# jaswon/osu-dreamer

Measured on AMD Instinct MI355X. Metric: denoiser train-steps/sec + 50-step sample latents/sec, 1/2/4/8 MI355X, higher is better.
Workload: dtype bf16

## Files before the change

### include/osu_dreamer_hip.h

```cpp
#ifndef OSU_DREAMER_HIP_H
#define OSU_DREAMER_HIP_H

#ifdef __cplusplus
extern "C" {
#endif

enum { OD_F32 = 0, OD_BF16 = 1,
       OD_F32X3 = 2,
       OD_F32X3W = 3,
       OD_F16 = 4 };
enum { OD_EPI_NONE = 0, OD_EPI_SILU = 1 };
enum { OD_ACT_NONE = 0, OD_ACT_SILU = 1 };
enum { OD_ERR_ARG = -1, OD_ERR_ALIGN = -2, OD_ERR_UNSUPPORTED = -3, OD_ERR_COMM = -4 };

int od_version(void);
const char* od_build_source_sha(void);
const char* od_error_string(int code);

int od_gemm_nt(int dtype, const void* A, int lda, const void* W, int ldw, const float* bias, void* C, int ldc,
               int M, int N, int K, int epilogue, int accumulate, void* stream);
int od_gemm_nt_qkrope(int dtype, const void* A, int lda, const void* W, int ldw, const float* bias, void* C, int ldc, int M,
                      int N, int K, const float* wq, const float* wk, const float* table, int L, int H, int hd, float eps,
                      float q_scale, void* stream);
int od_gemm_nt_qkrope_split(int dtype, const void* A, int lda, const void* W, int ldw, const float* bias, void* C, int ldc,
                            void* qk_out, int ldqk, int qk_dtype, int M, int N, int K, const float* wq, const float* wk, const float* table,
                            int L, int H, int hd, float eps, float q_scale, void* stream);
int od_gemm_tn(int dtype, const void* G, int ldg, const void* A, int lda, float* dW, int lddw, float* dbias, int M, int N,
               int K, void* stream);
int od_gemm_tn_blocks(int dtype, const void* G, int ldg, const void* A, int lda, float* dW, int lddw, float* dbias, int M, int N,
                      int K, int n_block, int n_valid, void* stream);
int od_colsum(int dtype, const void* G, int ldg, float* out, int M, int N, void* stream);
int od_pack_weight(int dtype, const float* src, int N, int K, void* dst, int Np, int Kp, int transpose,
                   const int* row_map, void* stream);

int od_linear_small(const float* x, const float* W, const float* b, float* out, float* pre, int B, int N, int K, int act,
                    void* stream);
int od_linear_small_bwd(const float* x, const float* W, const float* pre, const float* dout, float* dpre, float* dW,
                        float* db, float* dx, int accumulate_dx, int B, int N, int K, int act, void* stream);

int od_cl_to_frames(int dtype, const float* src, void* dst, int ldd, int B, int C, int L, void* stream);
int od_feed_gather(const float* store, long store_elems, const long* base, const long* cstride, const int* lens, float* out,
                   int N, int C, int Lpad, void* stream);
int od_proj_in(int dtype, const float* xt, const float* W, const float* bias, void* x, int ldx, int B, int E, int L,
               int D, void* stream);
int od_proj_in_bwd(int dtype, const float* xt, const void* dx, int ldx, float* dW, float* db, int B, int E, int L, int D,
                   void* stream);
int od_silu(int dtype, const void* x, void* y, long n, void* stream);
int od_silu_bwd(int dtype, const void* x, const void* dy, void* dx, long n, void* stream);

int od_rmsnorm_film(int dtype, const void* x, int ldx, const float* ssg, const void* cl, int ldcl, int cl_bcast,
                    void* h, int ldh, float* inv_rms, int B, int L, int C, float eps, void* stream);
int od_rmsnorm_film_bwd(int dtype, const void* x, int ldx, const float* inv_rms, const float* ssg, const void* dh,
                        int lddh, void* dres, int lddres, float* dssg, int B, int L, int C, void* stream);
int od_rmsnorm_gate_residual(int dtype, const void* x, int ldx, const void* h, int ldh, const float* ssg, void* xo,
                             int ldxo, float* inv_rms, int B, int L, int C, float eps, void* stream);
int od_rmsnorm_gate_residual_film(int dtype, const void* x, int ldx, const void* h, int ldh, const float* ssg_a, void* xo, int ldxo,
                                  float* inv_a, const float* ssg_b, const void* cl, int ldcl, int cl_bcast, void* h2, int ldh2,
                                  float* inv_b, int B, int L, int C, float eps, void* stream);
int od_rmsnorm_gate_residual_film_dwconv(int dtype, const void* x, int ldx, const void* h, int ldh, const float* ssg_a, void* xo, int ldxo,
                                         float* inv_a, const float* ssg_b, void* h2, int ldh2, float* inv_b, const float* conv_w,
                                         const float* conv_b, void* y, int ldy, int B, int L, int C, int ksize, float eps, void* stream);
int od_rmsnorm_gate_residual_bwd(int dtype, const void* h, int ldh, const float* inv_rms, const float* ssg,
                                 const void* dy, int lddy, void* dh, int lddh, float* dssg, int B, int L, int C,
                                 void* stream);

int od_rope_table(float* table, int L, int hd, void* stream);
int od_qk_norm_rope(int dtype, const void* qkv, int ldqkv, const float* wq, const float* wk, const float* table,
                    void* qk_out, int ldo, int B, int L, int H, int hd, float eps, float q_scale, void* stream);
int od_qk_norm_rope_bwd(int dtype, const void* qkv, int ldqkv, const float* wq, const float* wk, const float* table,
                        const void* dqk, int lddqk, void* dqkv, int lddqkv, float* dwq, float* dwk, int B, int L,
                        int H, int hd, float eps, float q_scale, void* stream);
int od_flash_attn_fwd(int dtype, const void* q, int ldq, const void* k, int ldk, const void* v, int ldv, void* o, int ldo,
                      float* lse, int B, int H, int L, int hd, float scale, int q_prescaled, void* stream);
int od_flash_attn_fwd_varlen(int dtype, const void* q, int ldq, const void* k, int ldk, const void* v, int ldv, void* o, int ldo,
                             float* lse, const int* lens, int B, int H, int L, int hd, float scale, int q_prescaled, void* stream);
int od_flash_attn_bwd(int dtype, const void* q, int ldq, const void* k, int ldk, const void* v, int ldv, const void* o,
                      int ldo, const void* dout, int lddo, const float* lse, float* delta, void* dq, int lddq, void* dk,
                      int lddk, void* dv, int lddv, int B, int H, int L, int hd, float scale, int q_prescaled, void* stream);
int od_attn_aux_create(void** aux_out);
int od_attn_aux_destroy(void* aux);
int od_flash_attn_bwd_aux(int dtype, const void* q, int ldq, const void* k, int ldk, const void* v, int ldv, const void* o,
                          int ldo, const void* dout, int lddo, const float* lse, float* delta, void* dq, int lddq, void* dk,
                          int lddk, void* dv, int lddv, int B, int H, int L, int hd, float scale, int q_prescaled, void* aux, void* stream);
int od_flash_attn_bwd_varlen(int dtype, const void* q, int ldq, const void* k, int ldk, const void* v, int ldv, const void* o,
                             int ldo, const void* dout, int lddo, const float* lse, float* delta, void* dq, int lddq, void* dk,
                             int lddk, void* dv, int lddv, const int* lens, int B, int H, int L, int hd, float scale, int q_prescaled,
                             void* aux, void* stream);
int od_flash_attn_bwd_fused_ws_bytes(int dtype, int B, int H, int L, long* total_out, long* zero_out);
int od_flash_attn_bwd_fused(int dtype, const void* q, int ldq, const void* k, int ldk, const void* v, int ldv, const void* o, int ldo,
                            const void* dout, int lddo, const float* lse, void* dq, int lddq, void* dk, int lddk, void* dv, int lddv,
                            int B, int H, int L, int hd, float scale, int q_prescaled, void* ws, long ws_bytes, void* stream);
int od_flash_attn_bwd_fused_status(const void* ws, int* err_out, void* stream);
int od_flash_attn_bwd_fused_err_offset(void);
int od_flash_attn_bwd_fused_passes(void);
int od_flash_attn_bwd_fused_prof(void* ws, long* out16);
int od_flash_attn_bwd_passes(void);

int od_dwconv(int dtype, const void* x, int ldx, const float* w, const float* bias, void* y, int ldy, int B, int L,
              int C, int ksize, void* stream);
int od_dwconv_varlen(int dtype, const void* x, int ldx, const float* w, const float* bias, void* y, int ldy, const int* lens,
                     int B, int L, int C, int ksize, void* stream);
int od_dwconv_bwd(int dtype, const void* x, int ldx, const float* w, const void* dy, int lddy, void* dx, int lddx,
                  float* dw, float* db, int B, int L, int C, int ksize, void* stream);
int od_dwconv_bwd_varlen(int dtype, const void* x, int ldx, const float* w, const void* dy, int lddy, void* dx, int lddx,
                         float* dw, float* db, const int* lens, int B, int L, int C, int ksize, void* stream);
int od_scale_channels(int dtype, void* x, int ldx, const float* scale, int B, int L, int C, void* stream);
int od_swiglu_rmsnorm(int dtype, const void* vg, int ldvg, void* hh, int ldhh, float* inv_rms, int M, int Hf, int Hp,
                      float eps, void* stream);
int od_swiglu_rmsnorm_bwd(int dtype, const void* vg, int ldvg, const float* inv_rms, const void* dhh, int lddhh,
                          void* dvg, int lddvg, int M, int Hf, int Hp, void* stream);

int od_final_norm_proj_out(int dtype, const void* x, int ldx, const float* W, const float* bias, float* v,
                           float* inv_rms, int B, int L, int C, int E, float eps, void* stream);
int od_final_norm_proj_out_bwd(int dtype, const void* x, int ldx, const float* inv_rms, const float* W, const float* dv,
                               void* dx, int lddx, float* dW, float* db, int B, int L, int C, int E, void* stream);
int od_uhead_fwd(const float* xt, const float* w0, const float* b0, const float* w1, const float* b1, const float* w3,
                 const float* b3, const float* w4, const float* b4, float* fsum, int B, int E, int L, int U,
// ... 157 lines not shown
```

### osu_dreamer_amd/csrc/rowops.hip

```cpp
#include "od_common.h"
#include "od_api_internal.h"

namespace {

#ifndef OD_QK_BPW
#define OD_QK_BPW 8
#endif
constexpr int ROWS_PER_WAVE_BWD = 16;

template <class T, int NCH>
__device__ __forceinline__ void load_row(const T* row, int C, int lane, float (&v)[NCH][8]) {
#pragma unroll
    for (int i = 0; i < NCH; i++) {
        const int c = (lane + 64 * i) * 8;
        if (c < C) od_ld8(row + c, v[i]);
        else {
#pragma unroll
            for (int e = 0; e < 8; e++) v[i][e] = 0.f;
        }
    }
}
template <int NCH>
__device__ __forceinline__ float row_sumsq(const float (&v)[NCH][8]) {
    float s = 0.f;
// ... 282 lines not shown
    const int b = blockIdx.y;
    const int l0 = (blockIdx.x * 4 + wave) * ROWS_PER_WAVE_BWD;
    float dg[NCH][8], gate[NCH][8];
#pragma unroll
    for (int i = 0; i < NCH; i++) {
        const int c = (lane + 64 * i) * 8;
#pragma unroll
        for (int e = 0; e < 8; e++) { dg[i][e] = 0.f; gate[i][e] = 0.f; }
        if (c < C) od_ld8(ssg + (size_t)b * 3 * C + 2 * C + c, gate[i]);
    }
    for (int r = 0; r < ROWS_PER_WAVE_BWD; r++) {
        const int l = l0 + r;
        if (l >= L) break;
        const long m = (long)b * L + l;
        float hv[NCH][8], gv[NCH][8];
        load_row<T, NCH>(h + m * ldh, C, lane, hv);
        load_row<T, NCH>(dy + m * lddy, C, lane, gv);
        const float inv = inv_rms[m];
        float dot = 0.f;
#pragma unroll
        for (int i = 0; i < NCH; i++)
#pragma unroll
            for (int e = 0; e < 8; e++) {
                const float hh = hv[i][e] * inv;
                dg[i][e] += gv[i][e] * hh;
                gv[i][e] *= gate[i][e];
                dot += gv[i][e] * hh;
                hv[i][e] = hh;
            }
        dot = od_wave_sum(dot) / (float)C;
#pragma unroll
        for (int i = 0; i < NCH; i++) {
            const int c = (lane + 64 * i) * 8;
            if (c >= C) continue;
            float o[8];
#pragma unroll
            for (int e = 0; e < 8; e++) o[e] = inv * (gv[i][e] - hv[i][e] * dot);
            od_st8(dh + m * lddh + c, o);
        }
    }
    for (int w = 0; w < 4; w++) {
        if (wave == w) {
#pragma unroll
            for (int i = 0; i < NCH; i++)
#pragma unroll
                for (int e = 0; e < 8; e++) {
                    const int idx = (lane + 64 * i) * 8 + e;
                    if (w == 0) red[idx] = dg[i][e]; else red[idx] += dg[i][e];
                }
        }
        __syncthreads();
    }
    for (int c = threadIdx.x; c < C; c += 256) od_red_add(det, dssg + (size_t)b * 3 * C + 2 * C + c, red[c]);
}

template <class T, int NCH>
__global__ __launch_bounds__(256) void swiglu_rmsnorm_kernel(const T* __restrict__ vg, int ldvg, T* __restrict__ hh, int ldhh,
                                                             float* __restrict__ inv_rms, long M, int Hf, int Hp, float eps) {
    const int lane = threadIdx.x & 63;
    const long m = (long)blockIdx.x * 4 + (threadIdx.x >> 6);
    if (m >= M) return;
    float v[NCH][8], g[NCH][8];
    load_row<T, NCH>(vg + m * ldvg, Hp, lane, v);
    load_row<T, NCH>(vg + m * ldvg + Hp, Hp, lane, g);
#pragma unroll
    for (int i = 0; i < NCH; i++)
#pragma unroll
        for (int e = 0; e < 8; e++) v[i][e] *= od_silu(g[i][e]);
    const float inv = rsqrtf(row_sumsq<NCH>(v) / (float)Hf + eps);
    if (lane == 0 && inv_rms) inv_rms[m] = inv;
#pragma unroll
    for (int i = 0; i < NCH; i++) {
        const int c = (lane + 64 * i) * 8;
        if (c >= Hp) continue;
        float o[8];
#pragma unroll
        for (int e = 0; e < 8; e++) o[e] = v[i][e] * inv;
        od_st8(hh + m * ldhh + c, o);
    }
}

template <class T, int NCH>
__global__ __launch_bounds__(256) void swiglu_rmsnorm_bwd_kernel(const T* __restrict__ vg, int ldvg, const float* __restrict__ inv_rms,
                                                                 const T* __restrict__ dhh, int lddhh, T* __restrict__ dvg, int lddvg,
                                                                 long M, int Hf, int Hp) {
    const int lane = threadIdx.x & 63;
    const long m = (long)blockIdx.x * 4 + (threadIdx.x >> 6);
    if (m >= M) return;
    float v[NCH][8], g[NCH][8], d[NCH][8];
    load_row<T, NCH>(vg + m * ldvg, Hp, lane, v);
    load_row<T, NCH>(vg + m * ldvg + Hp, Hp, lane, g);
    load_row<T, NCH>(dhh + m * lddhh, Hp, lane, d);
    const float inv = inv_rms[m];
    float dot = 0.f;
    float sg[NCH][8], gs[NCH][8];
#pragma unroll
    for (int i = 0; i < NCH; i++)
#pragma unroll
        for (int e = 0; e < 8; e++) {
            gs[i][e] = od_sigmoid(g[i][e]);
            sg[i][e] = g[i][e] * gs[i][e];
            dot += d[i][e] * (v[i][e] * sg[i][e] * inv);
        }
    dot = od_wave_sum(dot) / (float)Hf;
#pragma unroll
    for (int i = 0; i < NCH; i++) {
// ... 456 lines not shown
    DISPATCH_T_NCH(dtype, nch_for(C),
        OD_LAUNCH((rmsnorm_gate_res_kernel<T_, N_>), grid, dim3(256), 0, (hipStream_t)stream, (const T_*)x, ldx, (const T_*)h, ldh, ssg,
                  (T_*)xo, ldxo, inv_rms, B, L, C, eps));
    OD_CHECK_LAUNCH();
    return 0;
}

extern "C" int od_rmsnorm_gate_residual_film(int dtype, const void* x, int ldx, const void* h, int ldh, const float* ssg_a, void* xo,
                                             int ldxo, float* inv_a, const float* ssg_b, const void* cl, int ldcl, int cl_bcast,
                                             void* h2, int ldh2, float* inv_b, int B, int L, int C, float eps, void* stream) {
    if (C % 8 || ldx % 8 || ldh % 8 || ldxo % 8 || ldh2 % 8 || (cl && ldcl % 8)) return OD_ERR_ALIGN;
    const long M = (long)B * L;
    dim3 grid((unsigned)((M + 3) / 4));
    DISPATCH_T_NCH(dtype, nch_for(C),
        OD_LAUNCH((rmsnorm_gate_res_film_kernel<T_, N_>), grid, dim3(256), 0, (hipStream_t)stream, (const T_*)x, ldx, (const T_*)h, ldh,
                  ssg_a, (T_*)xo, ldxo, inv_a, ssg_b, (const T_*)cl, ldcl, cl_bcast, (T_*)h2, ldh2, inv_b, B, L, C, eps));
    OD_CHECK_LAUNCH();
    return 0;
}

extern "C" int od_rmsnorm_gate_residual_film_dwconv(int dtype, const void* x, int ldx, const void* h, int ldh, const float* ssg_a, void* xo,
                                                    int ldxo, float* inv_a, const float* ssg_b, void* h2, int ldh2, float* inv_b,
                                                    const float* conv_w, const float* conv_b, void* y, int ldy, int B, int L, int C,
                                                    int ksize, float eps, void* stream) {
    if (C % 8 || ldx % 8 || ldh % 8 || ldxo % 8 || (h2 && ldh2 % 8) || ldy % 8) return OD_ERR_ALIGN;
    if (C > 512 || (ksize != 3 && ksize != 5 && ksize != 7 && ksize != 9)) return OD_ERR_UNSUPPORTED;
    if (!x || !h || !xo || !y || !conv_w || !conv_b || xo == x || xo == h) return OD_ERR_ARG;
#ifndef OD_FD_SMALL_RUNS
#define OD_FD_SMALL_RUNS 2048
#endif
    const bool small = (long)B * ((L + 31) / 32) < OD_FD_SMALL_RUNS;
    const int run = small ? 8 : 32;
    dim3 grid((unsigned)((L + 4 * run - 1) / (4 * run)), (unsigned)B);
#define FD_GO2(T_, KS_, RUN_) OD_LAUNCH((rmsnorm_gate_res_film_dwconv_kernel<T_, KS_, RUN_>), grid, dim3(256), 0, (hipStream_t)stream, (const T_*)x, ldx, \
                   (const T_*)h, ldh, ssg_a, (T_*)xo, ldxo, inv_a, ssg_b, (T_*)h2, ldh2, inv_b, conv_w, conv_b, (T_*)y, ldy, B, L, C, eps)
#define FD_GO1(T_, KS_) do { if (small) FD_GO2(T_, KS_, 8); else FD_GO2(T_, KS_, 32); } while (0)
#define FD_GO(KS_) do { if (dtype == OD_BF16) FD_GO1(bf16_t, KS_); else if (dtype == OD_F32) FD_GO1(float, KS_); else return OD_ERR_UNSUPPORTED; } while (0)
    if (ksize == 5) FD_GO(5); else if (ksize == 3) FD_GO(3); else if (ksize == 7) FD_GO(7); else FD_GO(9);
#undef FD_GO
#undef FD_GO1
#undef FD_GO2
    OD_CHECK_LAUNCH();
    return 0;
}

extern "C" int od_rmsnorm_gate_residual_bwd(int dtype, const void* h, int ldh, const float* inv_rms, const float* ssg,
                                            const void* dy, int lddy, void* dh, int lddh, float* dssg, int B, int L, int C,
                                            void* stream) {
    if (C % 8 || ldh % 8 || lddy % 8 || lddh % 8) return OD_ERR_ALIGN;
    dim3 grid((L + 4 * ROWS_PER_WAVE_BWD - 1) / (4 * ROWS_PER_WAVE_BWD), B);
    DISPATCH_T_NCH(dtype, nch_for(C),
        OD_LAUNCH((rmsnorm_gate_res_bwd_kernel<T_, N_>), grid, dim3(256), 0, (hipStream_t)stream, (const T_*)h, ldh, inv_rms, ssg,
                  (const T_*)dy, lddy, (T_*)dh, lddh, dssg, B, L, C, od_det_active()));
    OD_CHECK_LAUNCH();
    return 0;
}

extern "C" int od_swiglu_rmsnorm(int dtype, const void* vg, int ldvg, void* hh, int ldhh, float* inv_rms, int M, int Hf, int Hp,
                                 float eps, void* stream) {
    if (Hp % 8 || ldvg % 8 || ldhh % 8 || Hf > Hp) return OD_ERR_ALIGN;
    dim3 grid((unsigned)((M + 3) / 4));
    DISPATCH_T_NCH(dtype, nch_for(Hp),
        OD_LAUNCH((swiglu_rmsnorm_kernel<T_, N_>), grid, dim3(256), 0, (hipStream_t)stream, (const T_*)vg, ldvg, (T_*)hh, ldhh, inv_rms,
                  (long)M, Hf, Hp, eps));
    OD_CHECK_LAUNCH();
    return 0;
}

extern "C" int od_swiglu_rmsnorm_bwd(int dtype, const void* vg, int ldvg, const float* inv_rms, const void* dhh, int lddhh,
                                     void* dvg, int lddvg, int M, int Hf, int Hp, void* stream) {
    if (Hp % 8 || ldvg % 8 || lddhh % 8 || lddvg % 8 || Hf > Hp) return OD_ERR_ALIGN;
    dim3 grid((unsigned)((M + 3) / 4));
    DISPATCH_T_NCH(dtype, nch_for(Hp),
        OD_LAUNCH((swiglu_rmsnorm_bwd_kernel<T_, N_>), grid, dim3(256), 0, (hipStream_t)stream, (const T_*)vg, ldvg, inv_rms,
                  (const T_*)dhh, lddhh, (T_*)dvg, lddvg, (long)M, Hf, Hp));
    OD_CHECK_LAUNCH();
    return 0;
}

extern "C" int od_final_norm_proj_out(int dtype, const void* x, int ldx, const float* W, const float* bias, float* v,
                                      float* inv_rms, int B, int L, int C, int E, float eps, void* stream) {
    if (C % 8 || ldx % 8) return OD_ERR_ALIGN;
    if (E > 8 || C > 1024) return OD_ERR_UNSUPPORTED;
    const long M = (long)B * L;
    dim3 grid((unsigned)((M + 3) / 4));
    DISPATCH_T_NCH(dtype, nch_for(C),
        OD_LAUNCH((final_proj_kernel<T_, N_>), grid, dim3(256), 0, (hipStream_t)stream, (const T_*)x, ldx, W, bias, v, inv_rms, B, L, C, E, eps));
    OD_CHECK_LAUNCH();
    return 0;
}

extern "C" int od_final_norm_proj_out_bwd(int dtype, const void* x, int ldx, const float* inv_rms, const float* W,
                                          const float* dv, void* dx, int lddx, float* dW, float* db, int B, int L, int C, int E,
                                          void* stream) {
    if (C % 8 || ldx % 8 || lddx % 8) return OD_ERR_ALIGN;
    if (E > 8 || C > 512) return OD_ERR_UNSUPPORTED;
    dim3 grid((L + 4 * ROWS_PER_WAVE_BWD - 1) / (4 * ROWS_PER_WAVE_BWD), B);
    if (dtype == OD_BF16)
        OD_LAUNCH((final_proj_bwd_kernel<bf16_t, 1>), grid, dim3(256), 0, (hipStream_t)stream, (const bf16_t*)x, ldx, inv_rms, W, dv,
                  (bf16_t*)dx, lddx, dW, db, B, L, C, E, od_det_active());
    else
        OD_LAUNCH((final_proj_bwd_kernel<float, 1>), grid, dim3(256), 0, (hipStream_t)stream, (const float*)x, ldx, inv_rms, W, dv,
                  (float*)dx, lddx, dW, db, B, L, C, E, od_det_active());
    OD_CHECK_LAUNCH();
    return 0;
}
// ... 80 lines not shown
```

### osu_dreamer_amd/engine.py

```python
from __future__ import annotations


import math
import os
from collections import OrderedDict
from typing import Dict, List, Optional

import torch

from . import det, ops
from ._lib import OD_ACT_NONE, OD_ACT_SILU

OD_FUSE_FILM_DWCONV_DEFAULT = "0"

FP32_EPS = float(torch.finfo(torch.float32).eps)

PLAN_CACHE_DEFAULT = 16
PLAN_CACHE_DETERMINISTIC = 2


def _ceil(x: int, m: int) -> int:
    return (x + m - 1) // m * m


# ... 246 lines not shown
                hdw = self.lbuf("hdw", i, (M, D))
                ops.rmsnorm_gate_residual_film_dwconv(x, ao, ssg1, x_mid, self.lbuf("inv2", i, (M,), f32), ssg2, h2 if self.train else None,
                                                      self.lbuf("inv3", i, (M,), f32),
                                                      self.P(p + "ffn.proj_vg.0.weight"), self.P(p + "ffn.proj_vg.0.bias"), hdw, B, L, self.ksize)
            else:
                ops.rmsnorm_gate_residual_film(x, ao, ssg1, x_mid, self.lbuf("inv2", i, (M,), f32), ssg2, None, False, h2,
                                               self.lbuf("inv3", i, (M,), f32), B, L)
            if fuse_dw:
                pass
            elif self.radius > 0:
                hdw = self.lbuf("hdw", i, (M, D))
                if self.varlen:
                    ops.dwconv_varlen(h2, self.P(p + "ffn.proj_vg.0.weight"), self.P(p + "ffn.proj_vg.0.bias"), hdw, self.ws.t["vl.lens"], B, L,
                                      self.ksize)
                else:
                    ops.dwconv(h2, self.P(p + "ffn.proj_vg.0.weight"), self.P(p + "ffn.proj_vg.0.bias"), hdw, B, L, self.ksize)
            else:
                hdw = h2
            vg = self.lbuf("vg", i, (M, 2 * Hp))
            ops.gemm_nt(hdw, self.W(p + "ffn.proj_vg.1"), self._packed[p + "ffn.proj_vg.1.b"], vg, x3=self.x3)
            hh = self.lbuf("hh", i, (M, Hp))
            ops.swiglu_rmsnorm(vg, hh, self.lbuf("inv4", i, (M,), f32), self.Hf, Hp)
            if self._drop_active():
                ops.scale_channels(hh, self.draw_dropout_mask(i), B, L)
            fo = self.lbuf("fo", i, (M, D))
            self.plain_gemm(hh, self.W(p + "ffn.proj_o"), self.P(p + "ffn.proj_o.bias"), fo)
            x = self.buf(f"x_in.{i + 1}", (M, D)) if self.train else self.buf(f"x_in.{(i + 1) & 1}", (M, D))
            if i + 1 < self.depth:
                h1 = self.lbuf("h1", i + 1, (M, D))
                ops.rmsnorm_gate_residual_film(x_mid, fo, ssg2, x, self.lbuf("inv5", i, (M,), f32),
                                               self.ws.t[f"ssg1.{i + 1}"], cl_of(i + 1), bcast, h1,
                                               self.lbuf("inv1", i + 1, (M,), f32), B, L)
            else:
                ops.rmsnorm_gate_residual(x_mid, fo, ssg2, x, self.lbuf("inv5", i, (M,), f32), B, L)
        self._x_last = x
        ops.final_norm_proj_out(x, self.P("proj_out.weight"), self.P("proj_out.bias"), v,
                                self.buf("invf", (M,), f32), B, L)
        fsum = self.buf("fsum", (B, self.U), f32)
        fsum.zero_()
        if self.varlen:
            ops.uhead_fwd_varlen(xt, self._uhead_w(), fsum, self.ws.t["vl.lens"], self.U)
            self._det_flush(fsum)
            ops.uhead_tail_varlen(fsum, self.ws.t["umod"], self.P("u_out.weight"), self.P("u_out.bias"), u, self.ws.t["vl.lens"], L,
                                  self.model.u_scale)
        else:
            ops.uhead_fwd(xt, self._uhead_w(), fsum, self.U)
            self._det_flush(fsum)
            ops.uhead_tail(fsum, self.ws.t["umod"], self.P("u_out.weight"), self.P("u_out.bias"), u, L, self.model.u_scale)

    def _v_of(self, qkv: torch.Tensor) -> torch.Tensor:
        v = qkv[:, 2 * self.dh:]
        return v.view(torch.float16) if self.attn_f16 else v

    def attn_bwd_passes(self) -> int:
        from . import _lib
        return int(_lib.lib().cdll.od_flash_attn_bwd_fused_passes() if self.fused_attn_bwd() else _lib.lib().cdll.od_flash_attn_bwd_passes())

    def fused_attn_bwd(self) -> bool:
        import os
        if self.dtype != torch.bfloat16 or self.hd != 64 or self.varlen:
            return False
        if self.attn_f16:
            return True
        env = os.environ.get("OD_ATTN_BWD_FUSED", "")
        if env in ("0", "1"):
            return env == "1"
        return self.L >= 2048

    def attn_bwd_launch(self, i: int, dy: torch.Tensor, delta: torch.Tensor, dqkv: torch.Tensor, core_only: bool = False):
        t, dh, p = self.ws.t, self.dh, f"net.layers.{i}."
        qk, qkv, y, lse = t[f"qk16.{i}" if self.attn_f16 else f"qk.{i}"], t[f"qkv.{i}"], t[f"y.{i}"], t[f"lse.{i}"]
        wq, wk = self.P(p + "attn.q_norm.weight"), self.P(p + "attn.k_norm.weight")
        gq, gk = self.G(p + "attn.q_norm.weight"), self.G(p + "attn.k_norm.weight")
        scale = 1.0 / math.sqrt(self.hd)
        dqk = self.buf("d.qk", (self.M, 2 * dh))
        if self.fused_attn_bwd():
            key = (self.B, self.H, self.L, qk.device, qk.dtype)
            ws = self._attn_ws_cache.get(key)
            if ws is None:
                if len(self._attn_ws_cache) >= 4:
                    self._attn_ws_cache.pop(next(iter(self._attn_ws_cache)))
                ws = self._attn_ws_cache[key] = ops.FusedAttnBwdWorkspace(self.B, self.H, self.L, qk.device, qk.dtype)
                ws.checked = False
            self._attn_ws = ws
            ops.flash_attn_bwd_fused(qk[:, :dh], qk[:, dh:], self._v_of(qkv), y, dy, lse, dqk[:, :dh], dqk[:, dh:], dqkv[:, 2 * dh:],
                                     self.B, self.H, self.L, self.hd, scale, self._attn_ws, q_prescaled=True)
        else:
            if (self._attn_aux is None or self._attn_aux.device != qk.device) and qk.is_cuda:
                if self._attn_aux is not None:
                    self._attn_aux.close()
                with torch.cuda.device(qk.device):
                    self._attn_aux = ops.AttnAux()
                self._attn_aux.device = qk.device
            if self.varlen:
                ops.flash_attn_bwd_varlen(qk[:, :dh], qk[:, dh:], qkv[:, 2 * dh:], y, dy, lse, delta, dqk[:, :dh], dqk[:, dh:],
                                          dqkv[:, 2 * dh:], self.ws.t["vl.lens"], self.B, self.H, self.L, self.hd, scale, q_prescaled=True,
                                          aux=self._attn_aux)
            else:
                ops.flash_attn_bwd(qk[:, :dh], qk[:, dh:], qkv[:, 2 * dh:], y, dy, lse, delta, dqk[:, :dh], dqk[:, dh:],
                                   dqkv[:, 2 * dh:], self.B, self.H, self.L, self.hd, scale, q_prescaled=True, aux=self._attn_aux)
        if not core_only:
            ops.qk_norm_rope_bwd(qkv, wq, wk, t["rope"], dqk, dqkv, gq, gk, self.B, self.L, self.H, self.hd, FP32_EPS, q_scale=self.q_scale)

    def _drop_active(self) -> bool:
        return self.dropout > 0.0 and self.model.training

    def _drop_mask(self, i: int) -> torch.Tensor:
        return self.ws.t[f"drop.{i}"]

    def draw_dropout_mask(self, i: int) -> torch.Tensor:
        keep = 1.0 - self.dropout
        m = self.buf(f"drop.{i}", (self.B, self.Hp), torch.float32)
        m.zero_()
        m[:, :self.Hf] = torch.empty(self.B, self.Hf, device=m.device, dtype=torch.float32).bernoulli_(keep) / keep
        return m

    def _uhead_w(self, grads=False):
        f = self.G if grads else self.P
        return [f(f"u_head.{j}.{s}") for j in (0, 1, 3, 4) for s in ("weight", "bias")]

    def backward(self, xt: torch.Tensor, style: torch.Tensor, du: torch.Tensor, dv: torch.Tensor, reducer=None):
        assert self.train
        B, L, M, D, dh, Hf, Hp, A = self.B, self.L, self.M, self.D, self.dh, self.Hf, self.Hp, self.A
        f32 = torch.float32
        dctx = det.context(self.model.arena.data.device)
        if dctx is not None:
            dctx.register(self.model.arena.ensure_grad())
        tab = self.ws.t["rope"]
        cg, a = self.ws.t["cg"], self.ws.t["a"]
        dx = self.buf("d.x", (M, D))
        dbr = self.buf("d.branch", (M, D))
        dtmp = self.buf("d.tmp", (M, D))
        dhh = self.buf("d.hh", (M, Hp))
        dvg = self.buf("d.vg", (M, 2 * Hp))
        dy = self.buf("d.y", (M, dh))
        dqkv = self.buf("d.qkv", (M, 3 * dh))
        da = self.buf("d.a", (self.Ma, A))
        delta = self.buf("d.delta", (B, self.H, L), f32)
        dcg = self.buf("d.cg", (B, self.Cg), f32)
        dssg1, dssg2 = self.buf("d.ssg1", (B, 3 * D), f32), self.buf("d.ssg2", (B, 3 * D), f32)

        ops.final_norm_proj_out_bwd(self._x_last, self.ws.t["invf"], self.P("proj_out.weight"), dv, dx,
                                    self.G("proj_out.weight"), self.G("proj_out.bias"), B, L)
        dfm, dmod = self.buf("d.fm", (B, self.U), f32), self.buf("d.mod", (B, 2 * self.U), f32)
        if self.varlen:
            lens = self.ws.t["vl.lens"]
            ops.uhead_tail_bwd_varlen(self.ws.t["fsum"], self.ws.t["umod"], self.P("u_out.weight"), self.P("u_out.bias"), du,
                                      dfm, dmod, self.G("u_out.weight"), self.G("u_out.bias"), lens, L, self.model.u_scale)
            ops.uhead_bwd_varlen(xt, self._uhead_w(), dfm, self._uhead_w(grads=True), lens, self.U)
        else:
            ops.uhead_tail_bwd(self.ws.t["fsum"], self.ws.t["umod"], self.P("u_out.weight"), self.P("u_out.bias"), du,
                               dfm, dmod, self.G("u_out.weight"), self.G("u_out.bias"), L, self.model.u_scale)
            ops.uhead_bwd(xt, self._uhead_w(), dfm, self._uhead_w(grads=True), self.U)
        ops.linear_small_bwd(cg, self.P("u_mod.weight"), None, dmod, self.buf("d.lin_pre_umod", (B, 2 * self.U), f32),
                             self.G("u_mod.weight"), self.G("u_mod.bias"), dcg, False, OD_ACT_NONE)
        self._det_flush_segment("tail")
        if reducer is not None:
            reducer.segment_done("tail")

        for i in reversed(range(self.depth)):
            p = f"net.layers.{i}."
            t = self.ws.t
            ssg1, ssg2 = t[f"ssg1.{i}"], t[f"ssg2.{i}"]
            dssg1.zero_()
            dssg2.zero_()
            ops.rmsnorm_gate_residual_bwd(t[f"fo.{i}"], t[f"inv5.{i}"], ssg2, dx, dbr, dssg2, B, L)
            ops.gemm_tn(dbr, t[f"hh.{i}"], self.G(p + "ffn.proj_o.weight"), n_cols=D, k_cols=Hf,
                        dbias=self.G(p + "ffn.proj_o.bias"))
            ops.gemm_nt(dbr, self.W(p + "ffn.proj_o", T=True), None, dhh)
            if self._drop_active():
                ops.scale_channels(dhh, self._drop_mask(i), B, L)
            ops.swiglu_rmsnorm_bwd(t[f"vg.{i}"], t[f"inv4.{i}"], dhh, dvg, Hf, Hp)
            gw, gb = self.G(p + "ffn.proj_vg.1.weight"), self.G(p + "ffn.proj_vg.1.bias")
            hdw = t[f"hdw.{i}"] if self.radius > 0 else t[f"h2.{i}"]
            ops.gemm_tn(dvg, hdw, gw, n_cols=2 * Hp, k_cols=D, dbias=gb, n_block=Hp, n_valid=Hf)
            if self.radius > 0:
                self.plain_gemm(dvg, self.W(p + "ffn.proj_vg.1", T=True), None, dtmp)
                if self.varlen:
                    ops.dwconv_bwd_varlen(t[f"h2.{i}"], self.P(p + "ffn.proj_vg.0.weight"), dtmp, dbr, self.G(p + "ffn.proj_vg.0.weight"),
                                          self.G(p + "ffn.proj_vg.0.bias"), self.ws.t["vl.lens"], B, L, self.ksize)
                else:
                    ops.dwconv_bwd(t[f"h2.{i}"], self.P(p + "ffn.proj_vg.0.weight"), dtmp, dbr,
                                   self.G(p + "ffn.proj_vg.0.weight"), self.G(p + "ffn.proj_vg.0.bias"), B, L, self.ksize)
            else:
                self.plain_gemm(dvg, self.W(p + "ffn.proj_vg.1", T=True), None, dbr)
            ops.rmsnorm_film_bwd(t[f"x_mid.{i}"], t[f"inv3.{i}"], ssg2, dbr, dx, dssg2, B, L)
            ops.rmsnorm_gate_residual_bwd(t[f"ao.{i}"], t[f"inv2.{i}"], ssg1, dx, dbr, dssg1, B, L)
            ops.gemm_tn(dbr, t[f"y.{i}"], self.G(p + "attn.out_proj.weight"), dbias=self.G(p + "attn.out_proj.bias"))
            ops.gemm_nt(dbr, self.W(p + "attn.out_proj", T=True), None, dy)
            self.attn_bwd_launch(i, dy, delta, dqkv)
            ops.gemm_tn(dqkv, t[f"h1.{i}"], self.G(p + "attn.qkv_proj.weight"), dbias=self.G(p + "attn.qkv_proj.bias"))
            self.plain_gemm(dqkv, self.W(p + "attn.qkv_proj", T=True), None, dtmp)
            ops.gemm_tn(dtmp, a, self.G(p + "proj_cl.weight"), dbias=self.G(p + "proj_cl.bias"))
            ops.gemm_nt(dtmp, self.W(p + "proj_cl", T=True), None, da, accumulate=(i != self.depth - 1))
            ops.rmsnorm_film_bwd(t[f"x_in.{i}"], t[f"inv1.{i}"], ssg1, dtmp, dx, dssg1, B, L)
            lp = self.buf("d.lin_pre_ssg", (B, 3 * D), f32)
            self._det_flush(dssg1, dssg2)
            ops.linear_small_bwd(cg, self.P(p + "ssg2.weight"), None, dssg2, lp, self.G(p + "ssg2.weight"),
                                 self.G(p + "ssg2.bias"), dcg, True, OD_ACT_NONE)
            ops.linear_small_bwd(cg, self.P(p + "ssg1.weight"), None, dssg1, lp, self.G(p + "ssg1.weight"),
                                 self.G(p + "ssg1.bias"), dcg, True, OD_ACT_NONE)
            self._det_flush_segment(f"layer{i}")
            if reducer is not None:
                reducer.segment_done(f"layer{i}")

        ops.proj_in_bwd(xt, dx, self.G("proj_in.weight"), self.G("proj_in.bias"))
        da_pre = self.buf("d.a_pre", (self.Ma, A))
        ops.silu_bwd(self.ws.t["a_pre"], da, da_pre)
        ops.gemm_tn(da_pre, self.ws.t["a_t"], self.G("proj_audio.0.weight"), dbias=self.G("proj_audio.0.bias"))
        self._det_flush(dcg)
        ops.linear_small_bwd(style, self.P("proj_style.0.weight"), self.ws.t["cg_pre"], dcg,
                             self.buf("d.lin_pre_style", (B, self.Cg), f32), self.G("proj_style.0.weight"),
                             self.G("proj_style.0.bias"), None, False, OD_ACT_SILU)
        self._det_flush_segment("head")
        if reducer is not None:
            reducer.segment_done("head")
        if self.fused_attn_bwd() and self._attn_ws is not None and not self._attn_ws.checked:
            self._attn_ws.checked = True
            self.check_attn_status()

    def attn_status_ptr(self) -> int:
        return self._attn_ws.err_ptr() if self._attn_ws is not None else 0

    def attn_status_view(self) -> torch.Tensor:
        return self._attn_ws.err_view()

    ATTN_STATUS = {1: "a launch left jobs unprocessed (an XCD ran none of its workgroups): gradients incomplete",
                   2: "a launch with another (B, H, L) than the workspace's earlier launches was refused",
                   3: "a chain wait ran out of time (the predecessor's write never came; OD_FB_CHAIN_TIMEOUT_MS): dq is NaN"}

    def check_attn_status(self):
        if self._attn_ws is None:
            return
        code = 0
        for ws in {id(w): w for w in [self._attn_ws, *self._attn_ws_cache.values()]}.values():
            code = code or ws.status()
        if code != 0:
            raise RuntimeError(f"od_flash_attn_bwd_fused status {code}: {self.ATTN_STATUS.get(code, '?')}; the optimizer steps since then "
                               "were skipped.  OD_ATTN_BWD_FUSED=0 selects the two-kernel backward.")
```

### osu_dreamer_amd/ops.py

```python
from __future__ import annotations

import os
from typing import Optional

import torch

from . import _lib
from ._lib import OD_ACT_NONE, OD_ACT_SILU, OD_BF16, OD_EPI_NONE, OD_EPI_SILU, OD_F32, OD_F32X3, OD_F32X3W


def dt_code(dtype: torch.dtype) -> int:
    if dtype == torch.float32:
        return OD_F32
    if dtype == torch.bfloat16:
        return OD_BF16
    if dtype == torch.float16:
        return _lib.OD_F16
    raise TypeError(f"unsupported compute dtype {dtype}")


class SplitWeight:

    def __init__(self, storage: torch.Tensor):
        self.t = storage
# ... 146 lines not shown


def silu(x, y):
    assert x.is_contiguous() and y.is_contiguous()
    _lib.lib().od_silu(dt_code(x.dtype), _p(x), _p(y), x.numel(), _stream(x))


def silu_bwd(x, dy, dx):
    assert x.is_contiguous() and dy.is_contiguous() and dx.is_contiguous()
    _lib.lib().od_silu_bwd(dt_code(x.dtype), _p(x), _p(dy), _p(dx), x.numel(), _stream(x))


def rmsnorm_film(x, ssg, cl, cl_bcast, h, inv_rms, B, L, eps=1e-6):
    C = x.shape[1]
    _f32(ssg, inv_rms)
    _lib.lib().od_rmsnorm_film(dt_code(x.dtype), _p(x), _ld(x), _p(ssg), _p(cl), _ld(cl) if cl is not None else 0,
                               int(cl_bcast), _p(h), _ld(h), _p(inv_rms), B, L, C, eps, _stream(x))


def rmsnorm_film_bwd(x, inv_rms, ssg, dh, dres, dssg, B, L):
    C = x.shape[1]
    _f32(ssg, inv_rms, dssg)
    _lib.lib().od_rmsnorm_film_bwd(dt_code(x.dtype), _p(x), _ld(x), _p(inv_rms), _p(ssg), _p(dh), _ld(dh), _p(dres),
                                   _ld(dres), _p(dssg), B, L, C, _stream(x))


def rmsnorm_gate_residual(x, h, ssg, xo, inv_rms, B, L, eps=1e-6):
    C = x.shape[1]
    _f32(ssg, inv_rms)
    _lib.lib().od_rmsnorm_gate_residual(dt_code(x.dtype), _p(x), _ld(x), _p(h), _ld(h), _p(ssg), _p(xo), _ld(xo),
                                        _p(inv_rms), B, L, C, eps, _stream(x))


def rmsnorm_gate_residual_film(x, h, ssg_a, xo, inv_a, ssg_b, cl, cl_bcast, h2, inv_b, B, L, eps=1e-6):
    _f32(ssg_a, ssg_b, inv_a, inv_b)
    _lib.lib().od_rmsnorm_gate_residual_film(dt_code(x.dtype), _p(x), _ld(x), _p(h), _ld(h), _p(ssg_a), _p(xo), _ld(xo),
                                             _p(inv_a), _p(ssg_b), _p(cl), _ld(cl) if cl is not None else 0, int(cl_bcast),
                                             _p(h2), _ld(h2), _p(inv_b), B, L, x.shape[1], eps, _stream(x))


def rmsnorm_gate_residual_film_dwconv(x, h, ssg_a, xo, inv_a, ssg_b, h2, inv_b, conv_w, conv_b, y, B, L, ksize, eps=1e-6):
    _f32(ssg_a, ssg_b, inv_a, inv_b, conv_w, conv_b)
    assert xo.data_ptr() != x.data_ptr() and xo.data_ptr() != h.data_ptr()
    _lib.lib().od_rmsnorm_gate_residual_film_dwconv(dt_code(x.dtype), _p(x), _ld(x), _p(h), _ld(h), _p(ssg_a), _p(xo), _ld(xo), _p(inv_a),
                                                    _p(ssg_b), _p(h2), _ld(h2) if h2 is not None else 0, _p(inv_b), _p(conv_w), _p(conv_b),
                                                    _p(y), _ld(y), B, L, x.shape[1], ksize, eps, _stream(x))


def rmsnorm_gate_residual_bwd(h, inv_rms, ssg, dy, dh, dssg, B, L):
    C = h.shape[1]
    _f32(ssg, inv_rms, dssg)
    _lib.lib().od_rmsnorm_gate_residual_bwd(dt_code(h.dtype), _p(h), _ld(h), _p(inv_rms), _p(ssg), _p(dy), _ld(dy),
                                            _p(dh), _ld(dh), _p(dssg), B, L, C, _stream(h))


def rope_table(table, L, hd):
    _f32(table)
    _lib.lib().od_rope_table(_p(table), L, hd, _stream(table))


def qk_norm_rope(qkv, wq, wk, table, qk_out, B, L, H, hd, eps, q_scale=1.0):
    _f32(wq, wk, table)
    _lib.lib().od_qk_norm_rope(dt_code(qkv.dtype), _p(qkv), _ld(qkv), _p(wq), _p(wk), _p(table), _p(qk_out),
                               _ld(qk_out), B, L, H, hd, eps, q_scale, _stream(qkv))


def qk_norm_rope_bwd(qkv, wq, wk, table, dqk, dqkv, dwq, dwk, B, L, H, hd, eps, q_scale=1.0):
    _f32(wq, wk, table, dwq, dwk)
    _lib.lib().od_qk_norm_rope_bwd(dt_code(qkv.dtype), _p(qkv), _ld(qkv), _p(wq), _p(wk), _p(table), _p(dqk), _ld(dqk),
                                   _p(dqkv), _ld(dqkv), _p(dwq), _p(dwk), B, L, H, hd, eps, q_scale, _stream(qkv))


def flash_attn_fwd(q, k, v, o, lse, B, H, L, hd, scale, x3=False, q_prescaled=False):
    _f32(lse)
    assert q.dtype == k.dtype == v.dtype and (o.dtype == q.dtype or (q.dtype == torch.float16 and o.dtype == torch.bfloat16))
    _lib.lib().od_flash_attn_fwd(mm_code(q.dtype, x3), _p(q), _ld(q), _p(k), _ld(k), _p(v), _ld(v), _p(o), _ld(o), _p(lse),
                                 B, H, L, hd, scale, int(q_prescaled), _stream(q))


class AttnAux:

    def __init__(self):
        import ctypes
        self.handle = ctypes.c_void_p()
        _lib.lib().od_attn_aux_create(ctypes.byref(self.handle))

    def close(self):
        if self.handle:
            _lib.lib().od_attn_aux_destroy(self.handle)
            self.handle = None

    def __del__(self):
        try:
            self.close()
        except Exception:
            pass


def flash_attn_fwd_varlen(q, k, v, o, lse, lens, B, H, L, hd, scale, x3=False, q_prescaled=False):
    _f32(lse)
    _i32(lens)
    assert q.dtype == k.dtype == v.dtype and (o.dtype == q.dtype or (q.dtype == torch.float16 and o.dtype == torch.bfloat16))
    _lib.lib().od_flash_attn_fwd_varlen(mm_code(q.dtype, x3), _p(q), _ld(q), _p(k), _ld(k), _p(v), _ld(v), _p(o), _ld(o), _p(lse),
                                        _p(lens), B, H, L, hd, scale, int(q_prescaled), _stream(q))


# ... 544 lines not shown
```

Baseline: 3.235.

## Fuse rmsnorm-FiLM backward with next gate-residual backward across layer boundaries

Adds a kernel that computes the FiLM rmsnorm backward (accumulating into the residual gradient) and then the following gate-residual rmsnorm backward in one pass. It is applied both inside each layer and across the boundary to the previous layer's FFN gate, which removes a separate kernel launch and a re-read of the residual gradient. The dwconv backward order is rearranged so the fused kernel can consume its output. The cost is more live registers and shared memory per block, restructured gradient-flush ordering, and the fused path is skipped for varlen.

Result: no change. 3.232, median of 2 (-0.1%).

```diff
diff --git a/include/osu_dreamer_hip.h b/include/osu_dreamer_hip.h
--- a/include/osu_dreamer_hip.h
+++ b/include/osu_dreamer_hip.h
@@ -63,6 +63,9 @@
 int od_rmsnorm_gate_residual_bwd(int dtype, const void* h, int ldh, const float* inv_rms, const float* ssg,
                                  const void* dy, int lddy, void* dh, int lddh, float* dssg, int B, int L, int C,
                                  void* stream);
+int od_rmsnorm_film_bwd_gate_residual_bwd(int dtype, const void* x, int ldx, const float* inv_a, const float* ssg_a, const void* dh,
+                                          int lddh, void* dres, int lddres, float* dssg_a, const void* hb, int ldhb, const float* inv_b,
+                                          const float* ssg_b, void* dbr, int lddbr, float* dssg_b, int B, int L, int C, void* stream);
 
 int od_rope_table(float* table, int L, int hd, void* stream);
 int od_qk_norm_rope(int dtype, const void* qkv, int ldqkv, const float* wq, const float* wk, const float* table,
diff --git a/osu_dreamer_amd/csrc/rowops.hip b/osu_dreamer_amd/csrc/rowops.hip
--- a/osu_dreamer_amd/csrc/rowops.hip
+++ b/osu_dreamer_amd/csrc/rowops.hip
@@ -358,6 +358,142 @@
         __syncthreads();
     }
     for (int c = threadIdx.x; c < C; c += 256) od_red_add(det, dssg + (size_t)b * 3 * C + 2 * C + c, red[c]);
+}
+
+template <class T> struct row8;
+template <> struct row8<bf16_t> { u32x4 r; };
+template <> struct row8<float> { float r[8]; };
+__device__ __forceinline__ void row8_load(row8<bf16_t>& w, const bf16_t* p) { w.r = *(const u32x4*)p; }
+__device__ __forceinline__ void row8_load(row8<float>& w, const float* p) { od_ld8(p, w.r); }
+__device__ __forceinline__ void row8_zero(row8<bf16_t>& w) { w.r = (u32x4)(0u); }
+__device__ __forceinline__ void row8_zero(row8<float>& w) {
+#pragma unroll
+    for (int e = 0; e < 8; e++) w.r[e] = 0.f;
+}
+__device__ __forceinline__ void row8_get(const row8<bf16_t>& w, float (&v)[8]) {
+#pragma unroll
+    for (int i = 0; i < 4; i++) {
+        union { uint32_t u; float f; } lo, hi;
+        lo.u = w.r[i] << 16; hi.u = w.r[i] & 0xffff0000u;
+        v[2 * i] = lo.f; v[2 * i + 1] = hi.f;
+    }
+}
+__device__ __forceinline__ void row8_get(const row8<float>& w, float (&v)[8]) {
+#pragma unroll
+    for (int e = 0; e < 8; e++) v[e] = w.r[e];
+}
+
+template <class T, int NCH>
+__global__ __launch_bounds__(256) void rmsnorm_film_bwd_gate_res_bwd_kernel(const T* __restrict__ x, int ldx, const float* __restrict__ inv_a,
+                                                                            const float* __restrict__ ssg_a, const T* __restrict__ dh, int lddh,
+                                                                            T* __restrict__ dres, int lddres, float* __restrict__ dssg_a,
+                                                                            const T* __restrict__ hb, int ldhb, const float* __restrict__ inv_b,
+                                                                            const float* __restrict__ ssg_b, T* __restrict__ dbr, int lddbr,
+                                                                            float* __restrict__ dssg_b, int B, int L, int C,
+                                                                            const OdDetTable* __restrict__ det) {
+    __shared__ float red[3][NCH * 512];
+    const int lane = threadIdx.x & 63, wave = threadIdx.x >> 6;
+    const int b = blockIdx.y;
+    const int l0 = (blockIdx.x * 4 + wave) * ROWS_PER_WAVE_BWD;
+    float dsc[NCH][8], dsh[NCH][8], dg[NCH][8], scl[NCH][8], gate[NCH][8];
+#pragma unroll
+    for (int i = 0; i < NCH; i++) {
+        const int c = (lane + 64 * i) * 8;
+#pragma unroll
+        for (int e = 0; e < 8; e++) { dsc[i][e] = 0.f; dsh[i][e] = 0.f; dg[i][e] = 0.f; scl[i][e] = 0.f; gate[i][e] = 0.f; }
+        if (c < C) {
+            od_ld8(ssg_a + (size_t)b * 3 * C + c, scl[i]);
+            od_ld8(ssg_b + (size_t)b * 3 * C + 2 * C + c, gate[i]);
+        }
+    }
+    constexpr bool PF = NCH == 1;
+    row8<T> px[NCH], pg[NCH], po[NCH], ph[NCH];
+    float pinv = 0.f, pinv2 = 0.f;
+    auto fetch = [&](int l) {
+        const long m = (long)b * L + l;
+#pragma unroll
+        for (int i = 0; i < NCH; i++) {
+            const int c = (lane + 64 * i) * 8;
+            if (c < C) {
+                row8_load(px[i], x + m * ldx + c); row8_load(pg[i], dh + m * lddh + c);
+                row8_load(po[i], dres + m * lddres + c); row8_load(ph[i], hb + m * ldhb + c);
+            } else { row8_zero(px[i]); row8_zero(pg[i]); row8_zero(po[i]); row8_zero(ph[i]); }
+        }
+        pinv = inv_a[m]; pinv2 = inv_b[m];
+    };
+    const int lend = l0 + ROWS_PER_WAVE_BWD < L ? l0 + ROWS_PER_WAVE_BWD : L;
+    if (PF && l0 < lend) fetch(l0);
+    for (int l = l0; l < lend; l++) {
+        const long m = (long)b * L + l;
+        if (!PF) fetch(l);
+        float xv[NCH][8], gv[NCH][8], hv[NCH][8], ov[NCH][8];
+#pragma unroll
+        for (int i = 0; i < NCH; i++) { row8_get(px[i], xv[i]); row8_get(pg[i], gv[i]); row8_get(po[i], ov[i]); row8_get(ph[i], hv[i]); }
+        const float inv = pinv, inv2 = pinv2;
+        if (PF && l + 1 < lend) fetch(l + 1);
+        float dot = 0.f;
+#pragma unroll
+        for (int i = 0; i < NCH; i++)
+#pragma unroll
+            for (int e = 0; e < 8; e++) {
+                const float xh = xv[i][e] * inv;
+                dsc[i][e] += gv[i][e] * xh;
+                dsh[i][e] += gv[i][e];
+                gv[i][e] *= (1.f + scl[i][e]);
+                dot += gv[i][e] * xh;
+                xv[i][e] = xh;
+            }
+        dot = od_wave_sum(dot) / (float)C;
+#pragma unroll
+        for (int i = 0; i < NCH; i++) {
+            const int c = (lane + 64 * i) * 8;
+            if (c >= C) continue;
+#pragma unroll
+            for (int e = 0; e < 8; e++) ov[i][e] += inv * (gv[i][e] - xv[i][e] * dot);
+            od_st8(dres + m * lddres + c, ov[i]);
+#pragma unroll
+            for (int e = 0; e < 8; e++) ov[i][e] = od_round_to<T>(ov[i][e]);
+        }
+        float dot2 = 0.f;
+#pragma unroll
+        for (int i = 0; i < NCH; i++)
+#pragma unroll
+            for (int e = 0; e < 8; e++) {
+                const float hh = hv[i][e] * inv2;
+                dg[i][e] += ov[i][e] * hh;
+                ov[i][e] *= gate[i][e];
+                dot2 += ov[i][e] * hh;
+                hv[i][e] = hh;
+            }
+        dot2 = od_wave_sum(dot2) / (float)C;
+#pragma unroll
+        for (int i = 0; i < NCH; i++) {
+            const int c = (lane + 64 * i) * 8;
+            if (c >= C) continue;
+            float o[8];
+#pragma unroll
+            for (int e = 0; e < 8; e++) o[e] = inv2 * (ov[i][e] - hv[i][e] * dot2);
+            od_st8(dbr + m * lddbr + c, o);
+        }
+    }
+    for (int w = 0; w < 4; w++) {
+        if (wave == w) {
+#pragma unroll
+            for (int i = 0; i < NCH; i++)
+#pragma unroll
+                for (int e = 0; e < 8; e++) {
+                    const int idx = (lane + 64 * i) * 8 + e;
+                    if (w == 0) { red[0][idx] = dsc[i][e]; red[1][idx] = dsh[i][e]; red[2][idx] = dg[i][e]; }
+                    else { red[0][idx] += dsc[i][e]; red[1][idx] += dsh[i][e]; red[2][idx] += dg[i][e]; }
+                }
+        }
+        __syncthreads();
+    }
+    for (int c = threadIdx.x; c < C; c += 256) {
+        od_red_add(det, dssg_a + (size_t)b * 3 * C + c, red[0][c]);
+        od_red_add(det, dssg_a + (size_t)b * 3 * C + C + c, red[1][c]);
+        od_red_add(det, dssg_b + (size_t)b * 3 * C + 2 * C + c, red[2][c]);
+    }
 }
 
 template <class T, int NCH>
@@ -920,6 +1056,21 @@
     DISPATCH_T_NCH(dtype, nch_for(C),
         OD_LAUNCH((rmsnorm_gate_res_bwd_kernel<T_, N_>), grid, dim3(256), 0, (hipStream_t)stream, (const T_*)h, ldh, inv_rms, ssg,
                   (const T_*)dy, lddy, (T_*)dh, lddh, dssg, B, L, C, od_det_active()));
+    OD_CHECK_LAUNCH();
+    return 0;
+}
+
+extern "C" int od_rmsnorm_film_bwd_gate_residual_bwd(int dtype, const void* x, int ldx, const float* inv_a, const float* ssg_a, const void* dh,
+                                                     int lddh, void* dres, int lddres, float* dssg_a, const void* hb, int ldhb,
+                                                     const float* inv_b, const float* ssg_b, void* dbr, int lddbr, float* dssg_b,
+                                                     int B, int L, int C, void* stream) {
+    if (C % 8 || ldx % 8 || lddh % 8 || lddres % 8 || ldhb % 8 || lddbr % 8) return OD_ERR_ALIGN;
+    if (!x || !dh || !dres || !hb || !dbr || dbr == dres || dbr == x || dbr == hb || dbr == dh) return OD_ERR_ARG;
+    dim3 grid((L + 4 * ROWS_PER_WAVE_BWD - 1) / (4 * ROWS_PER_WAVE_BWD), B);
+    DISPATCH_T_NCH(dtype, nch_for(C),
+        OD_LAUNCH((rmsnorm_film_bwd_gate_res_bwd_kernel<T_, N_>), grid, dim3(256), 0, (hipStream_t)stream, (const T_*)x, ldx, inv_a, ssg_a,
+                  (const T_*)dh, lddh, (T_*)dres, lddres, dssg_a, (const T_*)hb, ldhb, inv_b, ssg_b, (T_*)dbr, lddbr, dssg_b, B, L, C,
+                  od_det_active()));
     OD_CHECK_LAUNCH();
     return 0;
 }
diff --git a/osu_dreamer_amd/engine.py b/osu_dreamer_amd/engine.py
--- a/osu_dreamer_amd/engine.py
+++ b/osu_dreamer_amd/engine.py
@@ -322,6 +322,9 @@
         v = qkv[:, 2 * self.dh:]
         return v.view(torch.float16) if self.attn_f16 else v
 
+    def fused_hop_bwd(self) -> bool:
+        return not self.varlen and os.environ.get("OD_FUSE_FILM_DWCONV", "") != "0"
+
     def attn_bwd_passes(self) -> int:
         from . import _lib
         return int(_lib.lib().cdll.od_flash_attn_bwd_fused_passes() if self.fused_attn_bwd() else _lib.lib().cdll.od_flash_attn_bwd_passes())
@@ -428,13 +431,15 @@
         if reducer is not None:
             reducer.segment_done("tail")
 
+        hop = self.fused_hop_bwd()
         for i in reversed(range(self.depth)):
             p = f"net.layers.{i}."
             t = self.ws.t
             ssg1, ssg2 = t[f"ssg1.{i}"], t[f"ssg2.{i}"]
             dssg1.zero_()
-            dssg2.zero_()
-            ops.rmsnorm_gate_residual_bwd(t[f"fo.{i}"], t[f"inv5.{i}"], ssg2, dx, dbr, dssg2, B, L)
+            if not (hop and i < self.depth - 1):
+                dssg2.zero_()
+                ops.rmsnorm_gate_residual_bwd(t[f"fo.{i}"], t[f"inv5.{i}"], ssg2, dx, dbr, dssg2, B, L)
             ops.gemm_tn(dbr, t[f"hh.{i}"], self.G(p + "ffn.proj_o.weight"), n_cols=D, k_cols=Hf,
                         dbias=self.G(p + "ffn.proj_o.bias"))
             ops.gemm_nt(dbr, self.W(p + "ffn.proj_o", T=True), None, dhh)
@@ -444,18 +449,28 @@
             gw, gb = self.G(p + "ffn.proj_vg.1.weight"), self.G(p + "ffn.proj_vg.1.bias")
             hdw = t[f"hdw.{i}"] if self.radius > 0 else t[f"h2.{i}"]
             ops.gemm_tn(dvg, hdw, gw, n_cols=2 * Hp, k_cols=D, dbias=gb, n_block=Hp, n_valid=Hf)
-            if self.radius > 0:
-                self.plain_gemm(dvg, self.W(p + "ffn.proj_vg.1", T=True), None, dtmp)
-                if self.varlen:
-                    ops.dwconv_bwd_varlen(t[f"h2.{i}"], self.P(p + "ffn.proj_vg.0.weight"), dtmp, dbr, self.G(p + "ffn.proj_vg.0.weight"),
-                                          self.G(p + "ffn.proj_vg.0.bias"), self.ws.t["vl.lens"], B, L, self.ksize)
+            if hop:
+                if self.radius > 0:
+                    self.plain_gemm(dvg, self.W(p + "ffn.proj_vg.1", T=True), None, dbr)
+                    ops.dwconv_bwd(t[f"h2.{i}"], self.P(p + "ffn.proj_vg.0.weight"), dbr, dtmp,
+                                   self.G(p + "ffn.proj_vg.0.weight"), self.G(p + "ffn.proj_vg.0.bias"), B, L, self.ksize)
                 else:
-                    ops.dwconv_bwd(t[f"h2.{i}"], self.P(p + "ffn.proj_vg.0.weight"), dtmp, dbr,
-                                   self.G(p + "ffn.proj_vg.0.weight"), self.G(p + "ffn.proj_vg.0.bias"), B, L, self.ksize)
-            else:
-                self.plain_gemm(dvg, self.W(p + "ffn.proj_vg.1", T=True), None, dbr)
-            ops.rmsnorm_film_bwd(t[f"x_mid.{i}"], t[f"inv3.{i}"], ssg2, dbr, dx, dssg2, B, L)
-            ops.rmsnorm_gate_residual_bwd(t[f"ao.{i}"], t[f"inv2.{i}"], ssg1, dx, dbr, dssg1, B, L)
+                    self.plain_gemm(dvg, self.W(p + "ffn.proj_vg.1", T=True), None, dtmp)
+                ops.rmsnorm_film_bwd_gate_residual_bwd(t[f"x_mid.{i}"], t[f"inv3.{i}"], ssg2, dtmp, dx, dssg2,
+                                                       t[f"ao.{i}"], t[f"inv2.{i}"], ssg1, dbr, dssg1, B, L)
+            else:
+                if self.radius > 0:
+                    self.plain_gemm(dvg, self.W(p + "ffn.proj_vg.1", T=True), None, dtmp)
+                    if self.varlen:
+                        ops.dwconv_bwd_varlen(t[f"h2.{i}"], self.P(p + "ffn.proj_vg.0.weight"), dtmp, dbr, self.G(p + "ffn.proj_vg.0.weight"),
+                                              self.G(p + "ffn.proj_vg.0.bias"), self.ws.t["vl.lens"], B, L, self.ksize)
+                    else:
+                        ops.dwconv_bwd(t[f"h2.{i}"], self.P(p + "ffn.proj_vg.0.weight"), dtmp, dbr,
+                                       self.G(p + "ffn.proj_vg.0.weight"), self.G(p + "ffn.proj_vg.0.bias"), B, L, self.ksize)
+                else:
+                    self.plain_gemm(dvg, self.W(p + "ffn.proj_vg.1", T=True), None, dbr)
+                ops.rmsnorm_film_bwd(t[f"x_mid.{i}"], t[f"inv3.{i}"], ssg2, dbr, dx, dssg2, B, L)
+                ops.rmsnorm_gate_residual_bwd(t[f"ao.{i}"], t[f"inv2.{i}"], ssg1, dx, dbr, dssg1, B, L)
             ops.gemm_tn(dbr, t[f"y.{i}"], self.G(p + "attn.out_proj.weight"), dbias=self.G(p + "attn.out_proj.bias"))
             ops.gemm_nt(dbr, self.W(p + "attn.out_proj", T=True), None, dy)
             self.attn_bwd_launch(i, dy, delta, dqkv)
@@ -463,11 +478,17 @@
             self.plain_gemm(dqkv, self.W(p + "attn.qkv_proj", T=True), None, dtmp)
             ops.gemm_tn(dtmp, a, self.G(p + "proj_cl.weight"), dbias=self.G(p + "proj_cl.bias"))
             ops.gemm_nt(dtmp, self.W(p + "proj_cl", T=True), None, da, accumulate=(i != self.depth - 1))
-            ops.rmsnorm_film_bwd(t[f"x_in.{i}"], t[f"inv1.{i}"], ssg1, dtmp, dx, dssg1, B, L)
             lp = self.buf("d.lin_pre_ssg", (B, 3 * D), f32)
-            self._det_flush(dssg1, dssg2)
+            self._det_flush(dssg2)
             ops.linear_small_bwd(cg, self.P(p + "ssg2.weight"), None, dssg2, lp, self.G(p + "ssg2.weight"),
                                  self.G(p + "ssg2.bias"), dcg, True, OD_ACT_NONE)
+            if hop and i > 0:
+                dssg2.zero_()
+                ops.rmsnorm_film_bwd_gate_residual_bwd(t[f"x_in.{i}"], t[f"inv1.{i}"], ssg1, dtmp, dx, dssg1,
+                                                       t[f"fo.{i - 1}"], t[f"inv5.{i - 1}"], t[f"ssg2.{i - 1}"], dbr, dssg2, B, L)
+            else:
+                ops.rmsnorm_film_bwd(t[f"x_in.{i}"], t[f"inv1.{i}"], ssg1, dtmp, dx, dssg1, B, L)
+            self._det_flush(dssg1)
             ops.linear_small_bwd(cg, self.P(p + "ssg1.weight"), None, dssg1, lp, self.G(p + "ssg1.weight"),
                                  self.G(p + "ssg1.bias"), dcg, True, OD_ACT_NONE)
             self._det_flush_segment(f"layer{i}")
diff --git a/osu_dreamer_amd/ops.py b/osu_dreamer_amd/ops.py
--- a/osu_dreamer_amd/ops.py
+++ b/osu_dreamer_amd/ops.py
@@ -222,6 +222,14 @@
     _f32(ssg, inv_rms, dssg)
     _lib.lib().od_rmsnorm_gate_residual_bwd(dt_code(h.dtype), _p(h), _ld(h), _p(inv_rms), _p(ssg), _p(dy), _ld(dy),
                                             _p(dh), _ld(dh), _p(dssg), B, L, C, _stream(h))
+
+
+def rmsnorm_film_bwd_gate_residual_bwd(x, inv_a, ssg_a, dh, dres, dssg_a, hb, inv_b, ssg_b, dbr, dssg_b, B, L):
+    C = x.shape[1]
+    _f32(ssg_a, inv_a, dssg_a, ssg_b, inv_b, dssg_b)
+    _lib.lib().od_rmsnorm_film_bwd_gate_residual_bwd(dt_code(x.dtype), _p(x), _ld(x), _p(inv_a), _p(ssg_a), _p(dh), _ld(dh), _p(dres),
+                                                     _ld(dres), _p(dssg_a), _p(hb), _ld(hb), _p(inv_b), _p(ssg_b), _p(dbr), _ld(dbr),
+                                                     _p(dssg_b), B, L, C, _stream(x))
 
 
 def rope_table(table, L, hd):
```
